# canyagmur/XPoint

Measured on AMD Instinct MI355X. Metric: image-pairs/sec (detect+describe+match) 480x640 optical-thermal, higher is better.
Workload: dtype f32 (dense layers: f32 operands as 2 fp16 terms (operand error <= 2^-23, dropped cross term <= 2^-22: per product <= 2^-21 worst case, ~2^-25 typical), 3 fp16-MFMA partial products, f32 accumulate — GEMMs, implicit-GEMM convolutions and the fused block kernels alike; the deep-stage scan's dt project

## Files before the change

### include/xpoint_hip.h

```cpp
#ifndef XPOINT_HIP_H
#define XPOINT_HIP_H

#include <stddef.h>
#include <stdint.h>

#ifdef __cplusplus
extern "C" {
#endif

int xp_version(void);
const char* xp_last_error(void);
int xp_device_info(int device, int* cu_count, int* wave_size, char* arch, int arch_len);
int xp_knob_count(void);
int xp_knob_info(int index, const char** name, const char** where, const char** what);

int xp_selective_scan_fwd(const float* u, const float* delta, const float* A, const float* B, const float* C,
                          const float* D, const float* delta_bias, float* out, float* last_state,
                          int batch, int dim, int delta_dim, int seqlen, int dstate, int ngroups,
                          int delta_softplus, void* stream);

int xp_selective_scan_fwd_typed(const void* u, const void* delta, const float* A, const void* B, const void* C, const float* D,
                                const float* delta_bias, void* out, float* x_chunks, int itype, int out_float, int batch, int dim,
                                int delta_dim, int seqlen, int dstate, int ngroups, int delta_softplus, void* stream);

// ... 33 lines not shown

size_t xp_split_weights_x3_bytes(int N, int K);
int xp_split_weights_x3(const float* W, void* out, int N, int K, void* stream);
int xp_gemm_nt_x3(const float* A, const void* Wx3, float* C, const float* bias, const float* scale,
                  const float* shift, const float* res, int M, int N, int K, int lda, int ldc, int ldres, int act,
                  void* stream);
int xp_conv3x3_nhwc_x3(const float* x, const void* Wx3, float* y, const float* bias, const float* scale,
                       const float* shift, int batch, int Hi, int Wi, int Ci, int Co, int stride, int reflect_pad,
                       int act, void* stream);
size_t xp_split_weights_h2_bytes(int N, int K);
int xp_split_weights_h2(const float* W, void* out, int N, int K, void* stream);
int xp_gemm_nt_h2(const float* A, const void* Wh2, float* C, const float* bias, const float* scale, const float* shift,
                  const float* res, int M, int N, int K, int lda, int ldc, int ldres, int act, void* stream);
int xp_conv3x3_nhwc_h2(const float* x, const void* Wh2, float* y, const float* bias, const float* scale, const float* shift,
                       int batch, int Hi, int Wi, int Ci, int Co, int stride, int reflect_pad, int act, void* stream);
size_t xp_p32_bytes(int64_t M, int K);
int xp_split_activations_h2(const float* x, void* out_p32, int64_t M, int K, int ldx, void* stream);
int xp_gemm_nt_h2s_applies(int N, int K);
int xp_gemm_nt_h2s(const void* A_p32, const void* Wh2, void* C, int out_fmt, const float* bias, const float* scale, const float* shift,
                   const float* res, int M, int N, int K, int ldc, int ldres, int act, void* stream);
int xp_layernorm_p32(const float* x, void* y_p32, const float* w, const float* b, int64_t rows, int C, float eps, void* stream);
int xp_f32_to_f16(const float* x, void* y, int64_t n, void* stream);
int xp_gemm_nt_f16(const void* A, const void* W, void* C, int c_f32, const float* bias, const float* scale, const float* shift, const void* res,
                   int M, int N, int K, int lda, int ldc, int ldres, int act, void* stream);
int xp_conv3x3_nhwc_f16(const void* x, const void* W, void* y, int y_f32, const float* bias, const float* scale, const float* shift,
                        int batch, int Hi, int Wi, int Ci, int Co, int stride, int reflect_pad, int act, void* stream);

int xp_mlp_fused_f16_supported(int C, int H4);
int xp_mlp_fused_f16(const void* a, void* x, const void* W1, const float* b1, const void* W2, const float* b2, int M, int C, int H4, void* stream);
int xp_ln_mlp_fused_f16(void* x, const float* ln_w, const float* ln_b, float eps, const void* W1, const float* b1, const void* W2, const float* b2,
// ... 37 lines not shown
int xp_ln_proj_h2_pack(const void* W0h2, void* out, int C, int N, void* stream);
int xp_ln_proj_h2(const float* X, const float* ln_w, const float* ln_b, const void* Wpack, const void* W0h2, float* Out, int M, int C, int N,
                  float eps, void* stream);
size_t xp_ln_proj_x3_pack_bytes(int C, int N);
int xp_ln_proj_x3_pack(const void* W0x3, void* out, int C, int N, void* stream);
int xp_ln_proj_x3(const float* X, const float* ln_w, const float* ln_b, const void* Wpack, float* Out, int M, int C, int N,
                  float eps, void* stream);

int xp_layernorm(const float* x, float* y, const float* w, const float* b, int64_t rows, int C, float eps, int gelu,
                 void* stream);
int xp_dwconv3x3_silu(const float* x, const float* w9c, float* y, int batch, int H, int W, int C, void* stream);
int xp_stem_conv_ln_gelu(const float* img, const float* w9co, const float* bias, const float* ln_w, const float* ln_b,
                         float* y, int batch, int H, int W, int Co, float eps, void* stream);
int xp_depth_to_space_nhwc(const float* x, float* y, int batch, int H, int W, int C, int bs, void* stream);
int xp_softmax_shuffle(const float* logits, float* prob, int batch, int Hc, int Wc, int r, int ld, int mode, void* stream);
int xp_l2norm_rows(const float* x, float* y, int64_t rows, int C, float eps, void* stream);
int xp_nhwc_to_nchw(const float* x, float* y, int batch, int HW, int C, void* stream);
int xp_mul_mask(const float* x, const uint8_t* mask, float* y, int64_t n, void* stream);
int xp_stage_pair_batch(const float* optical, const float* thermal, float* images, const uint8_t* mask_optical,
                        const uint8_t* mask_thermal, uint8_t* masks, int64_t n, void* stream);
int xp_maxpool2_nhwc(const float* x, float* y, int batch, int H, int W, int C, void* stream);
int xp_costvolume_mean(const float* a, const float* b, float* v, int batch, int hw, int C, void* stream);
int xp_ingest_u8(const uint8_t* src, int H0, int W0, int channels, int top, int left, int h, int w,
                 const float* lut256, float* dst, void* stream);
int xp_u8_to_unit_f32(const uint8_t* src, float* dst, int64_t n, void* stream);
int xp_copy_to_mapped_host(const void* src_dev, void* dst_host, size_t bytes, void* stream);

typedef struct xp_model_cfg {
    int embed_dim;
    int n_stages;
// ... 111 lines not shown
```

### xpoint_amd/_lib.py

```python
from __future__ import annotations

import ctypes
import os

_HERE = os.path.dirname(os.path.abspath(__file__))
LIB_PATH = os.environ.get("XP_LIB_PATH") or os.path.join(_HERE, "libxpoint_hip.so")

_lib = None

c_p = ctypes.c_void_p
c_i = ctypes.c_int
c_f = ctypes.c_float
c_l = ctypes.c_int64


class XPointHipError(RuntimeError):
    pass


c_sz = ctypes.c_size_t
_SIGNATURES = {
    "xp_device_info": [c_i, ctypes.POINTER(c_i), ctypes.POINTER(c_i), ctypes.c_char_p, c_i],
    "xp_knob_info": [c_i, ctypes.POINTER(ctypes.c_char_p), ctypes.POINTER(ctypes.c_char_p), ctypes.POINTER(ctypes.c_char_p)],
    "xp_selective_scan_fwd": [c_p] * 9 + [c_i] * 7 + [c_p],
# ... 5 lines not shown
    "xp_ss2d_core_fwd": [c_p] * 10 + [c_sz] + [c_i] * 6 + [c_f, c_p],
    "xp_ss2d_core_set_mode": [c_i],
    "xp_set_dense_products": [c_i],
    "xp_set_dense_engine": [c_i],
    "xp_set_dense_override": [ctypes.c_uint64],
    "xp_set_amp_mode": [c_i],
    "xp_round_f16": [c_p, c_p, c_l, c_p],
    "xp_gemm_nt": [c_p] * 7 + [c_i] * 7 + [c_p],
    "xp_conv3x3_nhwc": [c_p] * 6 + [c_i] * 8 + [c_p],
    "xp_split_weights_x3": [c_p, c_p, c_i, c_i, c_p],
    "xp_gemm_nt_x3": [c_p] * 7 + [c_i] * 7 + [c_p],
    "xp_conv3x3_nhwc_x3": [c_p] * 6 + [c_i] * 8 + [c_p],
    "xp_split_weights_h2": [c_p, c_p, c_i, c_i, c_p],
    "xp_gemm_nt_h2": [c_p] * 7 + [c_i] * 7 + [c_p],
    "xp_conv3x3_nhwc_h2": [c_p] * 6 + [c_i] * 8 + [c_p],
    "xp_split_activations_h2": [c_p, c_p, c_l, c_i, c_i, c_p],
    "xp_gemm_nt_h2s": [c_p, c_p, c_p, c_i] + [c_p] * 4 + [c_i] * 6 + [c_p],
    "xp_layernorm_p32": [c_p] * 4 + [c_l, c_i, c_f, c_p],
    "xp_ss2d_core_fwd_ex": [c_p] * 9 + [c_i, c_p, c_sz] + [c_i] * 6 + [c_f, c_p],
    "xp_f32_to_f16": [c_p, c_p, c_l, c_p],
    "xp_gemm_nt_f16": [c_p, c_p, c_p, c_i] + [c_p] * 4 + [c_i] * 7 + [c_p],
    "xp_conv3x3_nhwc_f16": [c_p, c_p, c_p, c_i] + [c_p] * 3 + [c_i] * 8 + [c_p],
    "xp_mlp_fused_h2": [c_p] * 10 + [c_i] * 3 + [c_f, c_p],
    "xp_mlp_fused_h2_pack": [c_p] * 4 + [c_i] * 2 + [c_p],
    "xp_ln_proj_h2_pack": [c_p] * 2 + [c_i] * 2 + [c_p],
    "xp_ln_proj_h2": [c_p] * 6 + [c_i] * 3 + [c_f, c_p],
    "xp_mlp_fused_x3": [c_p] * 7 + [c_i] * 3 + [c_f, c_p],
    "xp_mlp_fused_x3_pack": [c_p] * 4 + [c_i] * 2 + [c_p],
    "xp_ln_proj_x3_pack": [c_p] * 2 + [c_i] * 2 + [c_p],
    "xp_ln_proj_x3": [c_p] * 5 + [c_i] * 3 + [c_f, c_p],
    "xp_layernorm": [c_p] * 4 + [c_l, c_i, c_f, c_i, c_p],
    "xp_dwconv3x3_silu": [c_p] * 3 + [c_i] * 4 + [c_p],
    "xp_stem_conv_ln_gelu": [c_p] * 6 + [c_i] * 4 + [c_f, c_p],
    "xp_depth_to_space_nhwc": [c_p] * 2 + [c_i] * 5 + [c_p],
    "xp_softmax_shuffle": [c_p] * 2 + [c_i] * 6 + [c_p],
    "xp_l2norm_rows": [c_p] * 2 + [c_l, c_i, c_f, c_p],
    "xp_nhwc_to_nchw": [c_p] * 2 + [c_i] * 3 + [c_p],
    "xp_mul_mask": [c_p] * 3 + [c_l, c_p],
    "xp_stage_pair_batch": [c_p] * 6 + [c_l, c_p],
    "xp_maxpool2_nhwc": [c_p] * 2 + [c_i] * 4 + [c_p],
    "xp_costvolume_mean": [c_p] * 3 + [c_i] * 3 + [c_p],
    "xp_ingest_u8": [c_p] + [c_i] * 7 + [c_p] * 3,
    "xp_u8_to_unit_f32": [c_p, c_p, c_l, c_p],
    "xp_copy_to_mapped_host": [c_p, c_p, c_sz, c_p],
    "xp_ctx_create": [c_p, ctypes.POINTER(c_p)],
    "xp_ctx_destroy": [c_p],
    "xp_param_info": [c_p, c_i, ctypes.c_char_p, c_i, ctypes.POINTER(c_sz), ctypes.POINTER(c_sz)],
    "xp_forward_shapes": [c_p, c_i, c_i, c_i, ctypes.POINTER(c_i), ctypes.POINTER(c_i), ctypes.POINTER(c_i)],
    "xp_xpoint_forward": [c_p, c_p, c_p, c_p, c_i, c_i, c_i, c_p, c_sz, c_p, c_p, c_p, c_p, c_p],
    "xp_xpoint_forward_ex": [c_p, c_p, c_p, c_p, c_i, c_i, c_i, c_p, c_sz, c_p, c_p, c_p, c_p, c_p, c_p],
# ... 36 lines not shown
    "xp_prof_get": [c_i, ctypes.c_char_p, c_i, ctypes.POINTER(ctypes.c_double), ctypes.POINTER(c_i),
                    ctypes.POINTER(ctypes.c_double), ctypes.POINTER(ctypes.c_double)],
}
_SIZE_QUERIES = {
    "xp_knob_count": (c_i, []),
    "xp_weights_numel": (c_sz, [c_p]),
    "xp_param_count": (c_i, [c_p]),
    "xp_forward_workspace_bytes": (c_sz, [c_p, c_i, c_i, c_i]),
    "xp_ss2d_core_workspace_bytes": (c_sz, [c_i] * 4),
    "xp_selective_scan_bwd_workspace_bytes": (c_sz, [c_i] * 6),
    "xp_descriptor_loss_workspace_bytes": (c_sz, [c_i] * 4),
    "xp_split_weights_x3_bytes": (c_sz, [c_i] * 2),
    "xp_split_weights_h2_bytes": (c_sz, [c_i] * 2),
    "xp_p32_bytes": (c_sz, [c_l, c_i]),
    "xp_gemm_nt_h2s_applies": (c_i, [c_i, c_i]),
    "xp_ss2d_core_p32_supported": (c_i, [c_i] * 4),
    "xp_split_weights_bytes": (c_sz, [c_p]),
    "xp_f16_weights_bytes": (c_sz, [c_p]),
    "xp_mlp_fused_f16_supported": (c_i, [c_i, c_i]),
    "xp_ss2d_core_f16_wants_f32_copies": (c_i, [c_i] * 4),
    "xp_mlp_fused_x3_supported": (c_i, [c_i, c_i]),
    "xp_get_dense_products": (c_i, []),
    "xp_get_dense_engine": (c_i, []),
    "xp_get_dense_override": (ctypes.c_uint64, []),
    "xp_get_amp_mode": (c_i, []),
    "xp_mlp_fused_x3_pack_bytes": (c_sz, [c_i, c_i, c_i]),
    "xp_mlp_fused_h2_pack_bytes": (c_sz, [c_i, c_i, c_i]),
    "xp_ln_proj_h2_pack_bytes": (c_sz, [c_i, c_i]),
    "xp_ln_proj_x3_pack_bytes": (c_sz, [c_i, c_i]),
    "xp_find_homography_workspace_bytes": (c_sz, [c_i]),
# ... 63 lines not shown
```

### xpoint_amd/csrc/elementwise.hip

```cpp
#include <stdlib.h>

#include <string>

#include <algorithm>

#include "xp_common.h"

namespace {

__global__ __launch_bounds__(256) void layernorm_kernel(const float* __restrict__ x, float* __restrict__ y,
                                                        const float* __restrict__ w, const float* __restrict__ b,
                                                        int64_t M, int C, float eps, int gelu) {
    const int lane = threadIdx.x & 63;
    const int64_t row = (int64_t)blockIdx.x * 4 + (threadIdx.x >> 6);
    if (row >= M) return;
    const float* xr = x + row * C;
    float v[16];
    float s = 0.f;
#pragma unroll
    for (int i = 0; i < 16; ++i) {
        const int c = lane + 64 * i;
        v[i] = (c < C) ? xr[c] : 0.f;
        s += v[i];
    }
// ... 485 lines not shown
    XpProfScope prof("depth_to_space", (hipStream_t)stream, 0.0, 8.0 * total);
    const bool vec = (C / (bs * bs)) % 4 == 0 && total < (1ll << 31) && ((((uintptr_t)x | (uintptr_t)y) & 15) == 0);
    if (vec) hipLaunchKernelGGL(depth_to_space_vec_kernel, dim3(xp_cdiv(total / 4, 256)), dim3(256), 0, (hipStream_t)stream, reinterpret_cast<const float4*>(x),
                                reinterpret_cast<float4*>(y), batch, H, W, C / 4, bs, limit, status);
    else hipLaunchKernelGGL(depth_to_space_kernel, dim3(xp_cdiv(total, 256)), dim3(256), 0, (hipStream_t)stream, x, y, batch, H, W, C, bs, limit, status);
    XP_LAUNCH_CHECK();
    return XP_OK;
}
extern "C" int xp_depth_to_space_nhwc(const float* x, float* y, int batch, int H, int W, int C, int bs, void* stream) {
    return xp_depth_to_space_nhwc_st(x, y, batch, H, W, C, bs, 0.f, nullptr, stream);
}

extern "C" int xp_softmax_shuffle(const float* logits, float* prob, int batch, int Hc, int Wc, int r, int ld, int mode, void* stream) {
    return xp_softmax_shuffle_st(logits, prob, batch, Hc, Wc, r, ld, mode, nullptr, stream);
}
int xp_softmax_shuffle_st(const float* logits, float* prob, int batch, int Hc, int Wc, int r, int ld, int mode, int* status, void* stream) {
    XP_CHECK_ARG(logits && prob, "xp_softmax_shuffle: null pointer");
    XP_CHECK_ARG(r * r + 1 <= 128 && ld >= r * r + 1, "xp_softmax_shuffle: r*r+1 must be <= 128 and <= ld");
    const int64_t cells = (int64_t)batch * Hc * Wc;
    XpProfScope prof("softmax_shuffle", (hipStream_t)stream, (double)cells * 4.0 * (r * r + 1), 4.0 * cells * (2.0 * r * r + 1));
    hipLaunchKernelGGL(softmax_shuffle_kernel, dim3(xp_cdiv(cells, 4 * SMX_CPW)), dim3(256), 0, (hipStream_t)stream, logits, prob, batch, Hc, Wc, r, ld, mode, status);
    XP_LAUNCH_CHECK();
    return XP_OK;
}

extern "C" int xp_l2norm_rows(const float* x, float* y, int64_t rows, int C, float eps, void* stream) {
    return xp_l2norm_rows_st(x, y, rows, C, eps, nullptr, stream);
}
int xp_l2norm_rows_st(const float* x, float* y, int64_t rows, int C, float eps, int* status, void* stream) {
    XP_CHECK_ARG(x && y, "xp_l2norm_rows: null pointer");
// ... 170 lines not shown
```

### xpoint_amd/csrc/gemm_h2.hip

```cpp
#include <stdlib.h>

#include <algorithm>
#include <string>

#include "gemm_h2_core.h"

bool xp_gemm_h2p_applies(const GemmParams& p);
int xp_gemm_h2p_launch(const GemmParams& p, hipStream_t s);

namespace {

__global__ __launch_bounds__(256) void h2_row_scale_kernel(const float* __restrict__ W, float* __restrict__ inv_scale, int N, int K) {
    const int n = blockIdx.x * 4 + (threadIdx.x >> 6);
    if (n >= N) return;
    const int lane = threadIdx.x & 63;
    float m = 0.f;
    for (int k = lane; k < K; k += 64) m = fmaxf(m, fabsf(W[(int64_t)n * K + k]));
    m = xp_wave_max(m);
    if (lane == 0) {
        int e = 0;
        if (m > 0.f && m < INFINITY) (void)frexpf(m, &e); else e = 14;
        e = e < -100 ? -100 : e;
        inv_scale[n] = ldexpf(1.f, e - 14);
    }
// ... 87 lines not shown
                iw = iw < 0 ? 0 : (iw >= p.Wi ? p.Wi - 1 : iw);
            }
            src = a_ptr[s] + ((int64_t)ih * p.Wi + iw) * p.Ci + ci;
        }
        v = *reinterpret_cast<const float4*>(src);
        return ok;
    };
    auto ldB = [&](int s, int t) -> uint4 { return w_unit[s][(t < nslab ? t : nslab - 1) * w_slab]; };

    f32x16 acc[TM][TN];
    T::run(lds_h2, p.K, ldA, ldB, acc);
    gemm_epilogue<T, TM, TN, true>(p, m0, n0, acc);
}

template <int TN, int MODE>
__global__ __launch_bounds__(256) void gemm_h2r_kernel(GemmParams p) {
    using T = GemmTileH2R<TN>;
    extern __shared__ __align__(16) unsigned char lds_h2[];
    const int ntn = (p.N + T::BN - 1) / T::BN;
    const int total = gridDim.x;
    const int bid = blockIdx.x, xcd = bid & 7, slot = bid >> 3;
    const int q = total >> 3, r = total & 7;
    const int logical = (xcd < r ? xcd * (q + 1) : r * (q + 1) + (xcd - r) * q) + slot;
    const int m0 = (logical / ntn) * T::BM, n0 = (logical % ntn) * T::BN;
    const int fh = (threadIdx.x & 63) >> 5;

    const int m = m0 + T::a_row();
    const int mc = m < p.M ? m : 0;
    const float* a_ptr;
    int a_oh = 0, a_ow = 0, a_tap[2] = {0, 0}, a_ci[2] = {0, 0};
    if (MODE == 0) a_ptr = p.A + (int64_t)mc * p.lda;
    else {
        const int hw = p.Ho * p.Wo;
        const int b = mc / hw, rr = mc - b * hw;
        a_oh = (rr / p.Wo) * p.stride - 1; a_ow = (rr % p.Wo) * p.stride - 1;
        a_ptr = p.A + (int64_t)b * p.Hi * p.Wi * p.Ci;
#pragma unroll
        for (int s = 0; s < 2; ++s) { const int k = s * 16 + fh * 8; a_tap[s] = k / p.Ci; a_ci[s] = k - a_tap[s] * p.Ci; }
    }
// ... 23 lines not shown
                ih = ih < 0 ? -ih : (ih >= p.Hi ? 2 * p.Hi - 2 - ih : ih);
                iw = iw < 0 ? -iw : (iw >= p.Wi ? 2 * p.Wi - 2 - iw : iw);
            } else {
                ok = ok && ih >= 0 && ih < p.Hi && iw >= 0 && iw < p.Wi;
                ih = ih < 0 ? 0 : (ih >= p.Hi ? p.Hi - 1 : ih);
                iw = iw < 0 ? 0 : (iw >= p.Wi ? p.Wi - 1 : iw);
            }
            src = a_ptr + ((int64_t)ih * p.Wi + iw) * p.Ci + ci;
        }
        lo = *reinterpret_cast<const float4*>(src);
        hi = *reinterpret_cast<const float4*>(src + 4);
        return ok;
    };
    auto ldB = [&](int s, int t) -> uint4 { return w_unit[s][(t < nslab ? t : nslab - 1) * w_slab]; };

    f32x16 acc[1][TN];
    T::run(lds_h2, p.K, ldA8, ldB, acc);
    gemm_epilogue<T, 1, TN, true>(p, m0, n0, acc);
}

template <int TN>
void launch_r(const GemmParams& p, hipStream_t s) {
    using T = GemmTileH2R<TN>;
    dim3 grid(xp_cdiv(p.N, T::BN) * xp_cdiv(p.M, T::BM));
    static const bool by_shape = getenv("XP_PROF_SHAPES") != nullptr;
    std::string tag = std::string(p.mode ? "conv3x3_h2r_mfma_" : "gemm_h2r_mfma_") + std::to_string(T::BM) + "x" + std::to_string(T::BN);
    if (by_shape) tag += "_M" + std::to_string(p.M) + "_N" + std::to_string(p.N) + "_K" + std::to_string(p.K) + (p.act == 1 ? "_gelu" : "");
    const double in_elems = p.mode == 0 ? (double)p.M * p.K : (double)p.M / (p.Ho * p.Wo) * p.Hi * p.Wi * p.Ci;
    XpProfScope prof(tag.c_str(), s, 2.0 * p.M * p.N * p.K, 4.0 * (in_elems + (double)p.N * p.K + (double)p.M * p.N * (p.res ? 2 : 1)));
    if (p.mode == 0) hipLaunchKernelGGL((gemm_h2r_kernel<TN, 0>), grid, dim3(T::NT), T::kLdsBytes, s, p);
    else hipLaunchKernelGGL((gemm_h2r_kernel<TN, 1>), grid, dim3(T::NT), T::kLdsBytes, s, p);
}

// ... 102 lines not shown
extern "C" int xp_conv3x3_nhwc_h2(const float* x, const void* Wh2, float* y, const float* bias, const float* scale, const float* shift,
                                  int batch, int Hi, int Wi, int Ci, int Co, int stride, int reflect_pad, int act, void* stream) {
    XP_CHECK_ARG(x && Wh2 && y, "xp_conv3x3_nhwc_h2: null pointer");
    XP_CHECK_ARG(Ci % 4 == 0, "xp_conv3x3_nhwc_h2: Ci must be a multiple of 4 (got %d)", Ci);
    XP_CHECK_ARG(stride == 1 || stride == 2, "xp_conv3x3_nhwc_h2: stride 1 or 2");
    XP_CHECK_ARG((scale == nullptr) == (shift == nullptr), "xp_conv3x3_nhwc_h2: scale and shift go together");
    XP_CHECK_ARG(!reflect_pad || (Hi >= 2 && Wi >= 2), "xp_conv3x3_nhwc_h2: reflection pad needs H,W >= 2");
    GemmParams p{};
    p.A = x; p.Wt = (const float*)Wh2; p.C = y; p.bias = bias; p.scale = scale; p.shift = shift; p.res = nullptr; p.wscale = h2_scales(Wh2, Co, 9 * Ci);
    p.Hi = Hi; p.Wi = Wi; p.Ci = Ci; p.stride = stride; p.reflect = reflect_pad;
    p.Ho = (Hi + 2 - 3) / stride + 1; p.Wo = (Wi + 2 - 3) / stride + 1;
    p.M = batch * p.Ho * p.Wo; p.N = Co; p.K = 9 * Ci; p.lda = 0; p.ldc = Co; p.ldres = 0; p.act = act; p.mode = 1;
    p.r16 = xp_amp_value();
    return dispatch(p, (hipStream_t)stream);
}
```

### xpoint_amd/csrc/model.cpp

```cpp
#include <math.h>
#include <stdlib.h>
#include <string.h>

#include <string>
#include <vector>

#include "xp_common.h"
#include "../../include/xpoint_hip.h"

namespace {

struct Param { std::string name; size_t offset; size_t numel; };
struct SplitW { std::string name; size_t src_offset; int N, K; size_t byte_offset, h2_offset, f16_offset; };
struct MlpPack { std::string block; int C, H4; size_t byte_offset, in_offset, h2_offset, h2_in_offset; };

struct Ctx {
    xp_model_cfg cfg;
    int nstages;
    int dims[4], ranks[4];
    std::vector<Param> params;
    std::vector<SplitW> split;
    std::vector<MlpPack> packs;
    size_t total, split_bytes, h2_bytes;
    size_t f16_bytes;
// ... 240 lines not shown
        return xp_gemm_nt(A, P(w), C, bias, scale, shift, res, M, N, K, lda, ldc, ldres, act, stream);
    };
    auto conv = [&](const float* x, const std::string& w, float* y, const float* bias, const float* scale, const float* shift,
                    int Hi, int Wi, int Ci, int Co, int stride, int reflect, int act, int id) -> int {
        if (wsplit && h2 && !ov(id)) return xp_conv3x3_nhwc_h2(x, (const char*)wsplit + c->h2_off(w), y, bias, scale, shift, batch, Hi, Wi, Ci, Co, stride, reflect, act, stream);
        if (wsplit) return xp_conv3x3_nhwc_x3(x, (const char*)wsplit + c->split_off(w), y, bias, scale, shift, batch, Hi, Wi, Ci, Co, stride, reflect, act, stream);
        return xp_conv3x3_nhwc(x, P(w), y, bias, scale, shift, batch, Hi, Wi, Ci, Co, stride, reflect, act, stream);
    };
    const float eps = 1e-5f;
    const int E = c->cfg.embed_dim;
    static const bool no_fused_mlp = getenv("XP_NO_FUSED_MLP") != nullptr && atoi(getenv("XP_NO_FUSED_MLP")) != 0;
    const bool amp = xp_amp_value() != 0;
    XP_CHECK_ARG(!amp || (wsplit && h2), "xp_xpoint_forward: the mixed-precision class (xp_set_amp_mode) runs on the split-fp16 engine: pass wsplit and "
                 "select xp_set_dense_engine(1) with xp_set_dense_products(6)");
    const bool fuse_mlp = wsplit != nullptr && !no_fused_mlp && !amp;
    static const int fuse_max_c = getenv("XP_FUSE_MAXC") ? atoi(getenv("XP_FUSE_MAXC")) : 1 << 30;
    static const bool fused_x3 = getenv("XP_FUSED_X3") != nullptr && atoi(getenv("XP_FUSED_X3")) != 0;

    RUN(xp_stem_conv_ln_gelu(images, P("stem.w"), P("stem.b"), P("stem.ln_w"), P("stem.ln_b"), HB, batch, H, W, E / 2, eps, stream));
    RUN(conv(HB, "pe2.w", T1, P("pe2.b"), nullptr, nullptr, sh.Hs, sh.Ws, E / 2, E, 2, 0, 0, 0));
    RUN(xp_layernorm(T1, X, P("pe2.ln_w"), P("pe2.ln_b"), sh.M[0], E, eps, 0, stream));

    for (int s = 0; s < c->nstages; ++s) {
        const int C = c->dims[s], R = c->ranks[s], H4 = (int)(C * c->cfg.mlp_ratio);
        const int M = (int)sh.M[s];
        const int XW = 4 * (R + 2);
        for (int j = 0; j < c->cfg.depths[s]; ++j) {
            const std::string b = "s" + std::to_string(s) + ".b" + std::to_string(j) + ".";
            const bool fused_block = fuse_mlp && C <= fuse_max_c && c->pack_off(b) != (size_t)-1;
            const int id0 = blk();
            const bool ring_ok = wsplit && h2 && !amp && !fused_block;
            const bool ring_in = ring_ok && xp_gemm_nt_h2s_applies(C, C) && !ov(id0);
            const bool ring_out = ring_ok && xp_gemm_nt_h2s_applies(C, C) && !ov(id0 + 2) && xp_ss2d_core_p32_supported(sh.H[s], sh.W[s], C, R);
            const bool ring_mlp = ring_ok && xp_gemm_nt_h2s_applies(H4, C) && xp_gemm_nt_h2s_applies(C, H4) && !ov(id0 + 3) && !ov(id0 + 4);
            const bool tail_x3 = ov(id0 + 2) || ov(id0 + 3) || ov(id0 + 4);
            const char* wb = (const char*)wsplit;
// ... 35 lines not shown
        if (s < c->nstages - 1) {
            const std::string d = "s" + std::to_string(s) + ".ds.";
            RUN(conv(X, d + "w", T1, P(d + "b"), nullptr, nullptr, sh.H[s], sh.W[s], C, 2 * C, 2, 0, 0, 41 + s));
            RUN(xp_layernorm(T1, X, P(d + "ln_w"), P(d + "ln_b"), sh.M[s + 1], 2 * C, eps, 0, stream));
        }
    }
    const int L = c->nstages - 1;
    RUN(xp_depth_to_space_nhwc_st(X, enc_nhwc, batch, sh.H[L], sh.W[L], c->dims[L], 4, (wsplit && h2 && !ov(44)) ? 65504.f : INFINITY, status, stream));

    const int EC = enc_channels_of(*c), HC = c->cfg.head_channels, DET = c->cfg.det_channels, DS = c->cfg.desc_size;
    const int Mc = batch * sh.Hc * sh.Wc;
    if (prob || logits_nhwc || desc_nhwc) {
        RUN(conv(enc_nhwc, "head.w", HB, P("head.b"), P("head.scale"), P("head.shift"), sh.Hc, sh.Wc, EC, 2 * HC, 1, 1, 2, 44));
    }
    if (prob || logits_nhwc) {
        float* lg = logits_nhwc ? logits_nhwc : T2;
        RUN(gemm(HB, "det2.w", lg, P("det2.b"), P("det2.scale"), P("det2.shift"), nullptr, Mc, DET, HC, 2 * HC, DET, 0, 0, 45));
        if (prob) RUN(xp_softmax_shuffle_st(lg, prob, batch, sh.Hc, sh.Wc, 8, DET, 0, status, stream));
    }
    if (desc_nhwc) {
        RUN(gemm(HB + HC, "desc2.w", T1, P("desc2.b"), P("desc2.scale"), P("desc2.shift"), nullptr, Mc, DS, HC, 2 * HC, DS, 0, 0, 46));
        RUN(xp_l2norm_rows_st(T1, desc_nhwc, Mc, DS, 1e-12f, status, stream));
    }
    return XP_OK;
}


extern "C" size_t xp_f16_weights_bytes(void* ctx) { return ctx ? ((Ctx*)ctx)->f16_bytes : 0; }

extern "C" int xp_prepare_f16_weights(void* ctx, const float* weights, void* w16, size_t w16_bytes, void* stream) {
    XP_CHECK_ARG(ctx && weights && w16, "xp_prepare_f16_weights: null pointer");
    Ctx* c = (Ctx*)ctx;
    XP_CHECK_ARG(w16_bytes >= c->f16_bytes, "xp_prepare_f16_weights: buffer too small");
// ... 104 lines not shown
```

### xpoint_amd/csrc/xp_knobs.h

```cpp
#pragma once

struct XpKnob { const char* name; const char* where; const char* what; };

static const XpKnob kXpKnobs[] = {
    {"XP_DENSE_ENGINE", "api.cpp", "initial value of xp_set_dense_engine: h2 (default) | x3"},
    {"XP_DENSE_PRODUCTS", "api.cpp", "initial value of xp_set_dense_products: 6 (default) | 3 | 1"},
    {"XP_RING", "gemm_ring.hip", "0: keep every layer on the round-4 GEMM kernels (default 1: ring engine for N, K >= 256 layers of the split class)"},
    {"XP_RING_TILE", "gemm_ring.hip", "force the ring tile: 0 = 256x256, 1 = 256x128, 2 = 128x128"},
    {"XP_H2P", "gemm_h2p.hip", "ping-pong split-fp16 GEMM: 0 off, 1 (default) K >= 768 and N >= 384, 2 widened"},
    {"XP_H2_ENGINE", "gemm_h2.hip", "rs | lds: force the row-stationary / tile variant of the split-fp16 GEMM"},
    {"XP_H2_TILE", "gemm_h2.hip", "force the split-fp16 tile (0..4)"},
    {"XP_H2_NO64", "gemm_h2.hip", "64x128 tile rule: 0 old, 1 never, 2 (default) only below 128 tiles"},
    {"XP_H2_NGROUP", "gemm_h2.hip", "column tiles per group of the tile order (0 = N-fastest)"},
    {"XP_X3_TILE", "gemm_x3.hip", "force the split-bf16 tile"},
    {"XP_GEMM_STAGGER", "gemm.hip", "exact-f32 GEMM: start-up delay (cycles) of the second workgroup slot of every CU"},
    {"XP_GEMM_STAMPS", "gemm.hip", "exact-f32 GEMM: s_memtime stamps per workgroup (debug)"},
    {"XP_F16_TILE", "gemm_f16.hip", "force the fp16-class tile (0..5)"},
    {"XP_F16_BK", "gemm_f16.hip", "force the fp16-class slab depth: 32 | 64"},
    {"XP_NO_FUSED_MLP", "model.cpp", "1: stages 0-1 as separate launches instead of xp_ln_proj + xp_mlp_fused"},
    {"XP_FUSE_MAXC", "model.cpp", "blocks wider than this many channels run unfused"},
    {"XP_FUSED_X3", "model.cpp", "1: fused block kernels on the x3 planes under the h2 engine"},
    {"XP_NO_LN_PROJ_F16", "model.cpp", "fp16 class: LayerNorm and in_proj as two launches"},
    {"XP_NO_FUSED_MLP_F16", "model.cpp", "fp16 class: 1 two-GEMM MLP everywhere, 2 fused MLP behind a separate LayerNorm"},
    {"XP_MLP_TAIL", "mlp_fused.hip", "0: no separate 4-wave launch for a last round less than half full (C = 192)"},
    {"XP_MLP_NW8", "mlp_fused.hip", "1: 8-wave workgroups in the x3 fused tail (C <= 96)"},
    {"XP_MLP_H2_NW4", "mlp_fused.hip", "1: 4-wave workgroups in the h2 fused tail at C = 192"},
    {"XP_SS2D_SEQ", "ss2d.hip", "0 / 1: force the chunked / sequential form of the fused SS2D core (also xp_ss2d_core_set_mode)"},
    {"XP_SS2D_SEQ_MAXL", "ss2d.hip", "L bound of the automatic choice of the sequential form (default 8192)"},
    {"XP_SS2D_SEQ_V1", "ss2d.hip", "1: first sequential kernel (dt projection on the vector ALU)"},
    {"XP_SS2D_SEQ_NW", "ss2d.hip", "waves per route of the pipelined sequential kernel: 1 | 2 | 4"},
    {"XP_SS2D_TBUDGET", "ss2d.hip", "chunk-length budget of the chunked passes (default 6144 pixel-channels)"},
    {"XP_SS2D_T", "ss2d.hip", "chunk length per channel count, e.g. \"96:32,192:16,384:16\""},
    {"XP_SS2D_THREADS", "ss2d.hip", "threads per workgroup of the chunked passes (default 192)"},
    {"XP_SCAN_V1", "selective_scan.hip", "force the first d_state = 1 operator-boundary scan kernel"},
// ... 22 lines not shown
```

Baseline: 1767.

## Fuse patch-embed LayerNorm and detector softmax-shuffle into h2 GEMM epilogues

Adds row-operation epilogues to the split-fp16 GEMM kernel. One applies LayerNorm across the 96 output channels of the pe2 conv in registers, and the other applies the 65-way detector softmax and depth-to-space shuffle directly after the det2 GEMM. This removes two separate launches and the intermediate logits round trip through global memory. In exchange it adds cross-lane reductions and scattered stores inside the GEMM kernel, and both paths apply only to fixed channel counts.

```diff
diff --git a/include/xpoint_hip.h b/include/xpoint_hip.h
--- a/include/xpoint_hip.h
+++ b/include/xpoint_hip.h
@@ -71,6 +71,12 @@
                   const float* res, int M, int N, int K, int lda, int ldc, int ldres, int act, void* stream);
 int xp_conv3x3_nhwc_h2(const float* x, const void* Wh2, float* y, const float* bias, const float* scale, const float* shift,
                        int batch, int Hi, int Wi, int Ci, int Co, int stride, int reflect_pad, int act, void* stream);
+int xp_conv3x3_nhwc_h2_ln_supported(int Ci, int Co);
+int xp_conv3x3_nhwc_h2_ln(const float* x, const void* Wh2, float* y, const float* bias, const float* ln_w, const float* ln_b, float eps,
+                          int batch, int Hi, int Wi, int Ci, int Co, int stride, int reflect_pad, void* stream);
+int xp_gemm_nt_h2_softmax_shuffle_supported(int N, int K, int lda);
+int xp_gemm_nt_h2_softmax_shuffle(const float* A, const void* Wh2, float* prob, float* logits, const float* bias, const float* scale,
+                                  const float* shift, int batch, int Hc, int Wc, int K, int lda, int* status, void* stream);
 size_t xp_p32_bytes(int64_t M, int K);
 int xp_split_activations_h2(const float* x, void* out_p32, int64_t M, int K, int ldx, void* stream);
 int xp_gemm_nt_h2s_applies(int N, int K);
@@ -138,6 +144,7 @@
                          float* y, int batch, int H, int W, int Co, float eps, void* stream);
 int xp_depth_to_space_nhwc(const float* x, float* y, int batch, int H, int W, int C, int bs, void* stream);
 int xp_softmax_shuffle(const float* logits, float* prob, int batch, int Hc, int Wc, int r, int ld, int mode, void* stream);
+int xp_softmax_shuffle_status(const float* logits, float* prob, int batch, int Hc, int Wc, int r, int ld, int mode, int* status, void* stream);
 int xp_l2norm_rows(const float* x, float* y, int64_t rows, int C, float eps, void* stream);
 int xp_nhwc_to_nchw(const float* x, float* y, int batch, int HW, int C, void* stream);
 int xp_mul_mask(const float* x, const uint8_t* mask, float* y, int64_t n, void* stream);
diff --git a/xpoint_amd/_lib.py b/xpoint_amd/_lib.py
--- a/xpoint_amd/_lib.py
+++ b/xpoint_amd/_lib.py
@@ -43,6 +43,8 @@
     "xp_split_weights_h2": [c_p, c_p, c_i, c_i, c_p],
     "xp_gemm_nt_h2": [c_p] * 7 + [c_i] * 7 + [c_p],
     "xp_conv3x3_nhwc_h2": [c_p] * 6 + [c_i] * 8 + [c_p],
+    "xp_conv3x3_nhwc_h2_ln": [c_p] * 6 + [c_f] + [c_i] * 7 + [c_p],
+    "xp_gemm_nt_h2_softmax_shuffle": [c_p] * 7 + [c_i] * 5 + [c_p, c_p],
     "xp_split_activations_h2": [c_p, c_p, c_l, c_i, c_i, c_p],
     "xp_gemm_nt_h2s": [c_p, c_p, c_p, c_i] + [c_p] * 4 + [c_i] * 6 + [c_p],
     "xp_layernorm_p32": [c_p] * 4 + [c_l, c_i, c_f, c_p],
@@ -63,6 +65,7 @@
     "xp_stem_conv_ln_gelu": [c_p] * 6 + [c_i] * 4 + [c_f, c_p],
     "xp_depth_to_space_nhwc": [c_p] * 2 + [c_i] * 5 + [c_p],
     "xp_softmax_shuffle": [c_p] * 2 + [c_i] * 6 + [c_p],
+    "xp_softmax_shuffle_status": [c_p] * 2 + [c_i] * 6 + [c_p, c_p],
     "xp_l2norm_rows": [c_p] * 2 + [c_l, c_i, c_f, c_p],
     "xp_nhwc_to_nchw": [c_p] * 2 + [c_i] * 3 + [c_p],
     "xp_mul_mask": [c_p] * 3 + [c_l, c_p],
@@ -129,6 +132,8 @@
     "xp_split_weights_h2_bytes": (c_sz, [c_i] * 2),
     "xp_p32_bytes": (c_sz, [c_l, c_i]),
     "xp_gemm_nt_h2s_applies": (c_i, [c_i, c_i]),
+    "xp_conv3x3_nhwc_h2_ln_supported": (c_i, [c_i, c_i]),
+    "xp_gemm_nt_h2_softmax_shuffle_supported": (c_i, [c_i, c_i, c_i]),
     "xp_ss2d_core_p32_supported": (c_i, [c_i] * 4),
     "xp_split_weights_bytes": (c_sz, [c_p]),
     "xp_f16_weights_bytes": (c_sz, [c_p]),
diff --git a/xpoint_amd/csrc/elementwise.hip b/xpoint_amd/csrc/elementwise.hip
--- a/xpoint_amd/csrc/elementwise.hip
+++ b/xpoint_amd/csrc/elementwise.hip
@@ -523,6 +523,9 @@
 extern "C" int xp_softmax_shuffle(const float* logits, float* prob, int batch, int Hc, int Wc, int r, int ld, int mode, void* stream) {
     return xp_softmax_shuffle_st(logits, prob, batch, Hc, Wc, r, ld, mode, nullptr, stream);
 }
+extern "C" int xp_softmax_shuffle_status(const float* logits, float* prob, int batch, int Hc, int Wc, int r, int ld, int mode, int* status, void* stream) {
+    return xp_softmax_shuffle_st(logits, prob, batch, Hc, Wc, r, ld, mode, status, stream);
+}
 int xp_softmax_shuffle_st(const float* logits, float* prob, int batch, int Hc, int Wc, int r, int ld, int mode, int* status, void* stream) {
     XP_CHECK_ARG(logits && prob, "xp_softmax_shuffle: null pointer");
     XP_CHECK_ARG(r * r + 1 <= 128 && ld >= r * r + 1, "xp_softmax_shuffle: r*r+1 must be <= 128 and <= ld");
diff --git a/xpoint_amd/csrc/gemm_h2.hip b/xpoint_amd/csrc/gemm_h2.hip
--- a/xpoint_amd/csrc/gemm_h2.hip
+++ b/xpoint_amd/csrc/gemm_h2.hip
@@ -4,6 +4,7 @@
 #include <string>
 
 #include "gemm_h2_core.h"
+#include "gemm_rowop.h"
 
 bool xp_gemm_h2p_applies(const GemmParams& p);
 int xp_gemm_h2p_launch(const GemmParams& p, hipStream_t s);
@@ -125,15 +126,14 @@
 }
 
 template <int TN, int MODE>
-__global__ __launch_bounds__(256) void gemm_h2r_kernel(GemmParams p) {
+__device__ __forceinline__ void h2r_accumulate(const GemmParams& p, unsigned char* lds_h2, int& m0, int& n0, f32x16 (&acc)[1][TN]) {
     using T = GemmTileH2R<TN>;
-    extern __shared__ __align__(16) unsigned char lds_h2[];
     const int ntn = (p.N + T::BN - 1) / T::BN;
     const int total = gridDim.x;
     const int bid = blockIdx.x, xcd = bid & 7, slot = bid >> 3;
     const int q = total >> 3, r = total & 7;
     const int logical = (xcd < r ? xcd * (q + 1) : r * (q + 1) + (xcd - r) * q) + slot;
-    const int m0 = (logical / ntn) * T::BM, n0 = (logical % ntn) * T::BN;
+    m0 = (logical / ntn) * T::BM; n0 = (logical % ntn) * T::BN;
     const int fh = (threadIdx.x & 63) >> 5;
 
     const int m = m0 + T::a_row();
@@ -187,9 +187,34 @@
     };
     auto ldB = [&](int s, int t) -> uint4 { return w_unit[s][(t < nslab ? t : nslab - 1) * w_slab]; };
 
+    T::run(lds_h2, p.K, ldA8, ldB, acc);
+}
+
+template <int TN, int MODE>
+__global__ __launch_bounds__(256) void gemm_h2r_kernel(GemmParams p) {
+    extern __shared__ __align__(16) unsigned char lds_h2[];
+    int m0, n0;
     f32x16 acc[1][TN];
-    T::run(lds_h2, p.K, ldA8, ldB, acc);
-    gemm_epilogue<T, 1, TN, true>(p, m0, n0, acc);
+    h2r_accumulate<TN, MODE>(p, lds_h2, m0, n0, acc);
+    gemm_epilogue<GemmTileH2R<TN>, 1, TN, true>(p, m0, n0, acc);
+}
+
+__global__ __launch_bounds__(256) void h2r_conv_ln_kernel(GemmParams p, RowOpParams q) {
+    extern __shared__ __align__(16) unsigned char lds_h2[];
+    int m0, n0;
+    f32x16 acc[1][3];
+    h2r_accumulate<3, 1>(p, lds_h2, m0, n0, acc);
+    rowop_pointwise<GemmTileH2R<3>, 3>(p, n0, acc);
+    rowop_layernorm96<GemmTileH2R<3>>(p, q, m0, acc);
+}
+
+__global__ __launch_bounds__(256) void h2r_gemm_softmax_shuffle_kernel(GemmParams p, RowOpParams q) {
+    extern __shared__ __align__(16) unsigned char lds_h2[];
+    int m0, n0;
+    f32x16 acc[1][3];
+    h2r_accumulate<3, 0>(p, lds_h2, m0, n0, acc);
+    rowop_pointwise<GemmTileH2R<3>, 3>(p, n0, acc);
+    rowop_softmax_shuffle65<GemmTileH2R<3>>(p, q, m0, acc);
 }
 
 template <int TN>
@@ -322,3 +347,55 @@
     p.r16 = xp_amp_value();
     return dispatch(p, (hipStream_t)stream);
 }
+
+extern "C" int xp_conv3x3_nhwc_h2_ln_supported(int Ci, int Co) { return Co == 96 && Ci > 0 && Ci % 8 == 0; }
+extern "C" int xp_gemm_nt_h2_softmax_shuffle_supported(int N, int K, int lda) { return N == 65 && K > 0 && K % 8 == 0 && lda >= K && lda % 4 == 0; }
+
+static void launch_rowop(bool conv, const GemmParams& p, const RowOpParams& q, double glue_bytes, hipStream_t s) {
+    using T = GemmTileH2R<3>;
+    const double in_elems = p.mode == 0 ? (double)p.M * p.K : (double)p.M / (p.Ho * p.Wo) * p.Hi * p.Wi * p.Ci;
+    XpProfScope prof(conv ? "h2r_conv_ln" : "h2r_gemm_softmax_shuffle", s, 2.0 * p.M * p.N * p.K, 4.0 * (in_elems + (double)p.N * p.K) + glue_bytes);
+    dim3 grid(xp_cdiv(p.M, T::BM));
+    if (conv) hipLaunchKernelGGL(h2r_conv_ln_kernel, grid, dim3(T::NT), T::kLdsBytes, s, p, q);
+    else hipLaunchKernelGGL(h2r_gemm_softmax_shuffle_kernel, grid, dim3(T::NT), T::kLdsBytes, s, p, q);
+}
+
+extern "C" int xp_conv3x3_nhwc_h2_ln(const float* x, const void* Wh2, float* y, const float* bias, const float* ln_w, const float* ln_b, float eps,
+                                     int batch, int Hi, int Wi, int Ci, int Co, int stride, int reflect_pad, void* stream) {
+    XP_CHECK_ARG(x && Wh2 && y && ln_w && ln_b, "xp_conv3x3_nhwc_h2_ln: null pointer");
+    XP_CHECK_ARG(xp_conv3x3_nhwc_h2_ln_supported(Ci, Co), "xp_conv3x3_nhwc_h2_ln: needs Co == 96 and Ci %% 8 == 0 (got Ci %d, Co %d)", Ci, Co);
+    XP_CHECK_ARG(batch > 0 && Hi > 0 && Wi > 0, "xp_conv3x3_nhwc_h2_ln: bad shape");
+    XP_CHECK_ARG(stride == 1 || stride == 2, "xp_conv3x3_nhwc_h2_ln: stride 1 or 2");
+    XP_CHECK_ARG(!reflect_pad || (Hi >= 2 && Wi >= 2), "xp_conv3x3_nhwc_h2_ln: reflection pad needs H,W >= 2");
+    XP_CHECK_ARG(!xp_amp_value(), "xp_conv3x3_nhwc_h2_ln: no mixed-precision form (xp_set_amp_mode): run xp_conv3x3_nhwc_h2 and xp_layernorm");
+    XP_CHECK_ARG((((uintptr_t)y | (uintptr_t)ln_w | (uintptr_t)ln_b) & 15) == 0, "xp_conv3x3_nhwc_h2_ln: y, ln_w and ln_b must be 16-byte aligned");
+    GemmParams p{};
+    p.A = x; p.Wt = (const float*)Wh2; p.C = y; p.bias = bias; p.wscale = h2_scales(Wh2, Co, 9 * Ci);
+    p.Hi = Hi; p.Wi = Wi; p.Ci = Ci; p.stride = stride; p.reflect = reflect_pad;
+    p.Ho = (Hi + 2 - 3) / stride + 1; p.Wo = (Wi + 2 - 3) / stride + 1;
+    p.M = batch * p.Ho * p.Wo; p.N = Co; p.K = 9 * Ci; p.ldc = Co; p.mode = 1;
+    RowOpParams q{};
+    q.ln_w = ln_w; q.ln_b = ln_b; q.eps = eps;
+    launch_rowop(true, p, q, 4.0 * p.M * p.N, (hipStream_t)stream);
+    XP_LAUNCH_CHECK();
+    return XP_OK;
+}
+
+extern "C" int xp_gemm_nt_h2_softmax_shuffle(const float* A, const void* Wh2, float* prob, float* logits, const float* bias, const float* scale,
+                                             const float* shift, int batch, int Hc, int Wc, int K, int lda, int* status, void* stream) {
+    const int N = 65;
+    XP_CHECK_ARG(A && Wh2 && prob, "xp_gemm_nt_h2_softmax_shuffle: null pointer");
+    XP_CHECK_ARG(batch > 0 && Hc > 0 && Wc > 0, "xp_gemm_nt_h2_softmax_shuffle: bad shape");
+    XP_CHECK_ARG(xp_gemm_nt_h2_softmax_shuffle_supported(N, K, lda), "xp_gemm_nt_h2_softmax_shuffle: needs K %% 8 == 0, lda >= K, lda %% 4 == 0 (got %d, %d)", K, lda);
+    XP_CHECK_ARG((scale == nullptr) == (shift == nullptr), "xp_gemm_nt_h2_softmax_shuffle: scale and shift go together");
+    XP_CHECK_ARG(!xp_amp_value(), "xp_gemm_nt_h2_softmax_shuffle: no mixed-precision form (xp_set_amp_mode): run xp_gemm_nt_h2 and xp_softmax_shuffle");
+    XP_CHECK_ARG((int64_t)batch * Hc * Wc < (1ll << 31) / 96, "xp_gemm_nt_h2_softmax_shuffle: too many cells");
+    GemmParams p{};
+    p.A = A; p.Wt = (const float*)Wh2; p.C = logits; p.bias = bias; p.scale = scale; p.shift = shift; p.wscale = h2_scales(Wh2, N, K);
+    p.M = batch * Hc * Wc; p.N = N; p.K = K; p.lda = lda; p.ldc = N; p.mode = 0;
+    RowOpParams q{};
+    q.prob = prob; q.Wc = Wc; q.status = status;
+    launch_rowop(false, p, q, 4.0 * p.M * (64 + (logits ? N : 0)), (hipStream_t)stream);
+    XP_LAUNCH_CHECK();
+    return XP_OK;
+}
diff --git a/xpoint_amd/csrc/gemm_rowop.h b/xpoint_amd/csrc/gemm_rowop.h
--- /dev/null
+++ b/xpoint_amd/csrc/gemm_rowop.h
@@ -0,0 +1,112 @@
+#pragma once
+#include "gemm_epilogue.h"
+
+struct RowOpParams {
+    const float* ln_w;
+    const float* ln_b;
+    float eps;
+    float* prob;
+    int Wc;
+    int* status;
+};
+
+__device__ __forceinline__ float rowop_swap16(float v) { return __int_as_float(__builtin_amdgcn_ds_swizzle(__float_as_int(v), 0x401F)); }
+
+template <class T, int TN>
+__device__ __forceinline__ void rowop_pointwise(const GemmParams& p, int n0, f32x16 (&acc)[1][TN]) {
+#pragma unroll
+    for (int j = 0; j < TN; ++j) {
+        const int cl = T::col_of(j);
+        const int clc = n0 + cl < p.N ? cl : 0;
+        const float bi = p.bias ? p.bias[n0 + clc] : 0.f;
+        const float ws = p.wscale[n0 + clc];
+        const float sc = p.scale ? p.scale[n0 + clc] : 1.f;
+        const float sh = p.shift ? p.shift[n0 + clc] : 0.f;
+#pragma unroll
+        for (int r = 0; r < 16; ++r) {
+            float v = acc[0][j][r] * ws + bi;
+            v = v * sc + sh;
+            acc[0][j][r] = 0.f + v;
+        }
+    }
+}
+
+template <class T>
+__device__ __forceinline__ void rowop_layernorm96(const GemmParams& p, const RowOpParams& q, int m0, f32x16 (&acc)[1][3]) {
+    const float fC = (float)p.N;
+    float w[3], b[3];
+#pragma unroll
+    for (int j = 0; j < 3; ++j) { w[j] = q.ln_w[T::col_of(j)]; b[j] = q.ln_b[T::col_of(j)]; }
+    float* cb = p.C + (int64_t)m0 * p.ldc;
+    auto butterfly = [](float s0, float s1, float s2) {
+        float t = (s0 + s2) + (s1 + 0.f);
+        t = t + rowop_swap16(t);
+        t = t + xp_dpp_mov<0x128>(t);
+        t = t + xp_dpp_mov<0x141>(t);
+        return t;
+    };
+#pragma unroll
+    for (int r = 0; r < 16; ++r) {
+        float s[3];
+#pragma unroll
+        for (int j = 0; j < 3; ++j) {
+            float a = acc[0][j][r];
+            a = a + xp_dpp_mov<0xB1>(a);
+            a = a + xp_dpp_mov<0x4E>(a);
+            s[j] = 0.f + a;
+        }
+        const float mean = butterfly(s[0], s[1], s[2]) / fC;
+#pragma unroll
+        for (int j = 0; j < 3; ++j) {
+            const float d = acc[0][j][r] - mean;
+            const float dx = xp_dpp_mov<0x00>(d), dy = xp_dpp_mov<0x55>(d), dz = xp_dpp_mov<0xAA>(d), dw = xp_dpp_mov<0xFF>(d);
+            float u = fmaf(dx, dx, 0.f);
+            u = fmaf(dy, dy, u); u = fmaf(dz, dz, u); u = fmaf(dw, dw, u);
+            s[j] = u;
+        }
+        const float rstd = 1.f / sqrtf(butterfly(s[0], s[1], s[2]) / fC + q.eps);
+        const int rl = T::row_of(0, r);
+        if (m0 + rl < p.M) {
+#pragma unroll
+            for (int j = 0; j < 3; ++j) cb[rl * p.ldc + T::col_of(j)] = (acc[0][j][r] - mean) * rstd * w[j] + b[j];
+        }
+    }
+}
+
+template <class T>
+__device__ __forceinline__ void rowop_softmax_shuffle65(const GemmParams& p, const RowOpParams& q, int m0, f32x16 (&acc)[1][3]) {
+    const int l31 = threadIdx.x & 31;
+    const bool has64 = l31 == 0;
+    int cell = m0 + T::row_of(0, 0);
+    int hb = cell / q.Wc, wc = cell - hb * q.Wc;
+    const int64_t Wf = (int64_t)q.Wc * 8;
+    const int pi = l31 >> 3, pj = l31 & 7;
+    bool bad = false;
+#pragma unroll
+    for (int r = 0; r < 16; ++r) {
+        const int rl = T::row_of(0, r);
+        const int step = r == 0 ? 0 : ((r & 3) + 8 * (r >> 2)) - (((r - 1) & 3) + 8 * ((r - 1) >> 2));
+        for (int k = 0; k < step; ++k) { ++wc; if (wc == q.Wc) { wc = 0; ++hb; } }
+        const bool rok = m0 + rl < p.M;
+        const float v0 = acc[0][0][r], v1 = acc[0][1][r], v2 = has64 ? acc[0][2][r] : -INFINITY;
+        if (p.C && rok) {
+            float* lg = p.C + (int64_t)(m0 + rl) * p.ldc;
+            lg[l31] = v0; lg[32 + l31] = v1;
+            if (has64) lg[64] = v2;
+        }
+        float ma = xp_row16_max(fmaxf(v0, v2)), mb = xp_row16_max(fmaxf(v1, -INFINITY));
+        const float mx = fmaxf(fmaxf(ma, rowop_swap16(ma)), fmaxf(mb, rowop_swap16(mb)));
+        float e0 = expf(v0 - mx), e1 = expf(v1 - mx);
+        const float e2 = has64 ? expf(v2 - mx) : 0.f;
+        const float ta = xp_row16_sum(e0 + e2), tb = xp_row16_sum(e1 + 0.f);
+        const float inv = 1.f / ((ta + rowop_swap16(ta)) + (tb + rowop_swap16(tb)));
+        e0 *= inv; e1 *= inv;
+        if (rok) {
+            bad = bad || !(inv <= 1.f);
+            float* pr = q.prob + ((int64_t)hb * 8 + pi) * Wf + wc * 8 + pj;
+            pr[0] = e0;
+            pr[4 * Wf] = e1;
+        }
+    }
+    if (q.status && bad && has64) atomicOr(q.status, XP_STATUS_PROB);
+}
diff --git a/xpoint_amd/csrc/model.cpp b/xpoint_amd/csrc/model.cpp
--- a/xpoint_amd/csrc/model.cpp
+++ b/xpoint_amd/csrc/model.cpp
@@ -278,12 +278,19 @@
     XP_CHECK_ARG(!amp || (wsplit && h2), "xp_xpoint_forward: the mixed-precision class (xp_set_amp_mode) runs on the split-fp16 engine: pass wsplit and "
                  "select xp_set_dense_engine(1) with xp_set_dense_products(6)");
     const bool fuse_mlp = wsplit != nullptr && !no_fused_mlp && !amp;
+    static const bool no_rowop = getenv("XP_NO_ROWOP_EPILOGUE") != nullptr && atoi(getenv("XP_NO_ROWOP_EPILOGUE")) != 0;
+    const bool rowop = wsplit != nullptr && h2 && !amp && !no_rowop;
+    auto aligned16 = [](const void* ptr) { return ((uintptr_t)ptr & 15) == 0; };
     static const int fuse_max_c = getenv("XP_FUSE_MAXC") ? atoi(getenv("XP_FUSE_MAXC")) : 1 << 30;
     static const bool fused_x3 = getenv("XP_FUSED_X3") != nullptr && atoi(getenv("XP_FUSED_X3")) != 0;
 
     RUN(xp_stem_conv_ln_gelu(images, P("stem.w"), P("stem.b"), P("stem.ln_w"), P("stem.ln_b"), HB, batch, H, W, E / 2, eps, stream));
-    RUN(conv(HB, "pe2.w", T1, P("pe2.b"), nullptr, nullptr, sh.Hs, sh.Ws, E / 2, E, 2, 0, 0, 0));
-    RUN(xp_layernorm(T1, X, P("pe2.ln_w"), P("pe2.ln_b"), sh.M[0], E, eps, 0, stream));
+    if (rowop && !ov(0) && xp_conv3x3_nhwc_h2_ln_supported(E / 2, E) && aligned16(X) && aligned16(P("pe2.ln_w")) && aligned16(P("pe2.ln_b"))) {
+        RUN(xp_conv3x3_nhwc_h2_ln(HB, (const char*)wsplit + c->h2_off("pe2.w"), X, P("pe2.b"), P("pe2.ln_w"), P("pe2.ln_b"), eps, batch, sh.Hs, sh.Ws, E / 2, E, 2, 0, stream));
+    } else {
+        RUN(conv(HB, "pe2.w", T1, P("pe2.b"), nullptr, nullptr, sh.Hs, sh.Ws, E / 2, E, 2, 0, 0, 0));
+        RUN(xp_layernorm(T1, X, P("pe2.ln_w"), P("pe2.ln_b"), sh.M[0], E, eps, 0, stream));
+    }
 
     for (int s = 0; s < c->nstages; ++s) {
         const int C = c->dims[s], R = c->ranks[s], H4 = (int)(C * c->cfg.mlp_ratio);
@@ -349,9 +356,14 @@
         RUN(conv(enc_nhwc, "head.w", HB, P("head.b"), P("head.scale"), P("head.shift"), sh.Hc, sh.Wc, EC, 2 * HC, 1, 1, 2, 44));
     }
     if (prob || logits_nhwc) {
-        float* lg = logits_nhwc ? logits_nhwc : T2;
-        RUN(gemm(HB, "det2.w", lg, P("det2.b"), P("det2.scale"), P("det2.shift"), nullptr, Mc, DET, HC, 2 * HC, DET, 0, 0, 45));
-        if (prob) RUN(xp_softmax_shuffle_st(lg, prob, batch, sh.Hc, sh.Wc, 8, DET, 0, status, stream));
+        if (prob && rowop && !ov(45) && xp_gemm_nt_h2_softmax_shuffle_supported(DET, HC, 2 * HC)) {
+            RUN(xp_gemm_nt_h2_softmax_shuffle(HB, (const char*)wsplit + c->h2_off("det2.w"), prob, logits_nhwc, P("det2.b"), P("det2.scale"), P("det2.shift"),
+                                              batch, sh.Hc, sh.Wc, HC, 2 * HC, status, stream));
+        } else {
+            float* lg = logits_nhwc ? logits_nhwc : T2;
+            RUN(gemm(HB, "det2.w", lg, P("det2.b"), P("det2.scale"), P("det2.shift"), nullptr, Mc, DET, HC, 2 * HC, DET, 0, 0, 45));
+            if (prob) RUN(xp_softmax_shuffle_st(lg, prob, batch, sh.Hc, sh.Wc, 8, DET, 0, status, stream));
+        }
     }
     if (desc_nhwc) {
         RUN(gemm(HB + HC, "desc2.w", T1, P("desc2.b"), P("desc2.scale"), P("desc2.shift"), nullptr, Mc, DS, HC, 2 * HC, DS, 0, 0, 46));
diff --git a/xpoint_amd/csrc/xp_knobs.h b/xpoint_amd/csrc/xp_knobs.h
--- a/xpoint_amd/csrc/xp_knobs.h
+++ b/xpoint_amd/csrc/xp_knobs.h
@@ -18,6 +18,7 @@
     {"XP_F16_TILE", "gemm_f16.hip", "force the fp16-class tile (0..5)"},
     {"XP_F16_BK", "gemm_f16.hip", "force the fp16-class slab depth: 32 | 64"},
     {"XP_NO_FUSED_MLP", "model.cpp", "1: stages 0-1 as separate launches instead of xp_ln_proj + xp_mlp_fused"},
+    {"XP_NO_ROWOP_EPILOGUE", "model.cpp", "1: patch-embed LayerNorm and detector softmax as launches of their own instead of the row-operation epilogues (gemm_rowop.h)"},
     {"XP_FUSE_MAXC", "model.cpp", "blocks wider than this many channels run unfused"},
     {"XP_FUSED_X3", "model.cpp", "1: fused block kernels on the x3 planes under the h2 engine"},
     {"XP_NO_LN_PROJ_F16", "model.cpp", "fp16 class: LayerNorm and in_proj as two launches"},
```

After: 1783, median of 6. No clear change (+0.9%).
